# evoldoers/historian

Hardware: AMD Instinct MI355X
Metric: forward-DP cells/s (higher is better)
Workload: dtype f64; 1 GPU; batch of independent 2x2000-residue protein leaf-profile pairs, WAG, t=0.2/0.3, full (unbanded) Forward DP; scaled-probability recursion with the reference's truncation: every pairwise sum of the reference's left-nested log_sum_exp drops a term that is at most e^-10 of the other, as the reference's table does (src/logsumexp.h:45); no table, log-probabilities at the store; lpEnd within 1e-9 rel. of; pairs_per_gpu=512, pairs_total=512, parallelism=pairs farmed across 1 rank(s); RCCL broadcast of model constants only

## Files before the change

historian_amd/csrc/hx_band2.hip:

```cpp
#include <hip/hip_runtime.h>
#include <cstdlib>
#include "hx_device.h"
#include "hx_lse.h"
#include "hx_common.h"
#include "hx_policy.h"
#include "hx_kernels.h"
#include "hx_bandedge.h"

namespace hx {

namespace {

typedef double d2v __attribute__((ext_vector_type(2)));
typedef int i2v __attribute__((ext_vector_type(2)));

#define HXB2_EMIN (-(1 << 28))
#define HXB2_LOG_ENTRIES 1536
#define HXB2_HOLE_BEGIN 16
#define HXB2_HOLE_END 16384
#define HXB2_W 32
#define HXB2_INFLIGHT 30
#define HXB2_LONG_ROW 16

struct L5 { double imm, imd, idm, imi, iiw; int e; };
__device__ __forceinline__ L5 l5_zero() { return L5{0., 0., 0., 0., 0., HXB2_EMIN}; }

__device__ __forceinline__ int ror1(int v) { return __builtin_amdgcn_mov_dpp(v, 0x13C , 0xf, 0xf, false); }
__device__ __forceinline__ int rot(const int, const int v) { return ror1(ror1(v)); }
__device__ __forceinline__ double rot(const int addr, const double v) {
  return __hiloint2double(rot(addr, __double2hiint(v)), rot(addr, __double2loint(v)));
}
__device__ __forceinline__ double ror1(const double v) { return __hiloint2double(ror1(__double2hiint(v)), ror1(__double2loint(v))); }
__device__ __forceinline__ L5 rot(const int, const L5& c) {
  const L5 t{ror1(c.imm), ror1(c.imd), ror1(c.idm), ror1(c.imi), ror1(c.iiw), ror1(c.e)};
  __builtin_amdgcn_sched_barrier(0);
  const L5 r{ror1(t.imm), ror1(t.imd), ror1(t.idm), ror1(t.imi), ror1(t.iiw), ror1(t.e)};
  __builtin_amdgcn_sched_barrier(0);
  return r;
}

__device__ __forceinline__ double trunc_sum(double a, double b) {
  const double hi = fmax_plain(a, b), lo = fmin_plain(a, b);
  const int keep = lo > hi * 4.5399929762484854e-05 ? __double2hiint(lo) : 0;
  return hi + __hiloint2double(keep, __double2loint(lo));
}
template <bool TRUNC> __device__ __forceinline__ double lin_acc(double m, double p, double acc) {
  if (TRUNC) return trunc_sum(acc, m * p);
  return __builtin_fma(m, p, acc);
}

__device__ __forceinline__ double log_scaled(double m, int e) {
  const double f = __builtin_amdgcn_frexp_mant(m);
  const int k = __builtin_amdgcn_frexp_exp(m);
  const unsigned byte_off = ((unsigned)__double2hiint(f) >> 7) & 0x7FF0u;
  const d2v ce = *(const HX_LDS d2v*)(uintptr_t)byte_off;
  const double r = __builtin_fma(f, ce.x, -1.0);
  double p = __builtin_fma(r, 1.0 / 3.0, -0.5);
  p = __builtin_fma(p, r, 1.0);
  const double lf = __builtin_fma(p, r, ce.y);
  return __builtin_fma((double)(e + k), 0.693147180559945309417, lf);
}

__device__ __forceinline__ double read_lane(double v, int l) {
  return __hiloint2double(__builtin_amdgcn_readlane(__double2hiint(v), l), __builtin_amdgcn_readlane(__double2loint(v), l));
}

struct Band2Plan { int sbase, ycol, yclass, xclass, elds, stride, in_hole, total; };

__device__ __forceinline__ int block_offset(const Band2Plan& p, const int pair) {
  return pair < p.in_hole ? HXB2_HOLE_BEGIN + pair * p.stride : 16 * HXB2_LOG_ENTRIES + (pair - p.in_hole) * p.stride;
}

template <bool TRUNC, int DIR>
__global__ void __launch_bounds__(256)
k_band2_edges(const DevJob* __restrict__ jobs, const int n_jobs, const int write_edges) {
  const int lane = threadIdx.x & 63;
  const int job = (int)blockIdx.x * 4 + (int)(threadIdx.x >> 6);
  if (job >= n_jobs) return;
  const DevJob J = jobs[job];
  const int Re = J.n_rows, Ce = J.n_cols;
  const int nse = (Re + 63) >> 6;
  const int64_t plane = J.plane;
  const int blk = J.blk;
  HX_GLOBAL double* __restrict__ M = as_global(DIR ? J.bwd : J.fwd);
  const HX_GLOBAL i2v* xrecG = (const HX_GLOBAL i2v*)as_global(reinterpret_cast<const i2v*>(DIR ? J.band_rows_bwd : J.band_rows));
  if (DIR == 1) {
    const int64_t ssd = J.strip_stride;
    const int lo_last = reinterpret_cast<const int*>(reinterpret_cast<const i2v*>(J.band_rows_bwd) + (Re + 64))[nse];
    auto put_inf = [&](const int ip, const int jp) {
      const int64_t sl = cell_slot_blk(ssd, blk, ip, jp);
      M[sl] = HX_NEG_INF; M[plane + sl] = HX_NEG_INF; M[2 * plane + sl] = HX_NEG_INF; M[3 * plane + sl] = HX_NEG_INF;
      M[4 * plane + sl] = HX_NEG_INF;
    };
    if (write_edges) {
      for (int ip = 1 + lane; ip < Re; ip += 64) {
        const i2v rec = xrecG[ip];
        if ((rec.x & 0xFFFF) + ((rec.y >> 9) & 7) - ip > 0) put_inf(ip, 0);
      }
      for (int jp = 1 + lane; jp < lo_last; jp += 64) put_inf(Re - 1, jp);
    }
    {
      const i2v rec = xrecG[0];
      if (lane == 0 && (rec.x & 0xFFFF) + ((rec.y >> 9) & 7) > 0) {
        const double lpe = J.x.pack[4 * (size_t)Re] + J.y.pack[4 * (size_t)Ce];
        const int64_t sl = cell_slot_blk(ssd, blk, 0, 0);
        for (int st = 0; st < 5; ++st) M[st * plane + sl] = lpe + J.T[st][5];
      }
    }
  } else {
    const int own0 = (xrecG[0].x >> 16) & 0xFFFF;
    const i2v rec1 = xrecG[1];
    const bool row1_edge = ((rec1.x & 0xFFFF) + ((rec1.x >> 16) & 0xFFFF) - 1) < Ce - 1;
    const double T02 = J.T[0][2], T03 = J.T[0][3], T22 = J.T[2][2], T33 = J.T[3][3];
    const double pen0 = J.x.pack[3];
    double d_idm = HX_NEG_INF, d_imi = HX_NEG_INF;
    if (own0 < Ce - 1 || row1_edge) {
      const bool packed = J.strip_base != nullptr;
      const int w0 = packed ? J.fwd_windows[0] : 0, w1 = packed ? J.fwd_windows[1] : 0, w2 = packed ? J.fwd_windows[2] : 0,
                w3 = packed ? J.fwd_windows[3] : 0;
      const int64_t b0 = packed ? J.strip_base[0] : 0, b1 = packed ? J.strip_base[1] : 0;
      auto row0_slot = [&](const int j) -> int64_t {
        if (!packed) return cell_slot_blk(J.strip_stride, J.blk, 0, j);
        if (j >= w0 && j < w1) return b0 + ((int64_t)((j - w0) >> 1) << 7) + (j & 1);
        if (j >= w2 && j < w3) return b1 + ((int64_t)((j - w2) >> 1) << 7) + (j & 1);
        return -1;
      };
      const HX_GLOBAL double* ypack = as_global(J.y.pack);
      int full_from = own0 + 1;
      for (int l = 1; l < 4 && l < Re; ++l) {
        const i2v r = xrecG[l];
        if ((r.x & 0xFFFF) != 0xFFFF) full_from = max(full_from, (r.x & 0xFFFF) + ((r.x >> 16) & 0xFFFF) + 1);
      }
      full_from = (full_from + 1) & ~1;
      double carry_idm = 0., carry_imi = 0.;
      for (int j0 = 0; j0 < Ce; j0 += 64) {
        const int j = j0 + lane;
        const size_t jl = 4 * (size_t)(j < Ce ? j : Ce - 1);
        const double lrs = ypack[jl + 1], lin = ypack[jl + 2];
        double kidm, kimi;
        row0_chain_block(j0, lane, Ce, lrs, lin, T02, T03, T22, T33, pen0, carry_idm, carry_imi, kidm, kimi);
        if (Ce - 2 >= j0 && Ce - 2 < j0 + 64) { d_idm = read_lane(kidm, Ce - 2 - j0); d_imi = read_lane(kimi, Ce - 2 - j0); }
#pragma unroll
        for (int half = 0; half < 2; ++half) {
          const int line = (lane >> 2) + 16 * half, piece = lane & 3;
          const int je = j0 + 2 * line;
          const double e_idm = __shfl(kidm, 2 * line, 64), o_idm = __shfl(kidm, 2 * line + 1, 64);
          const double e_imi = __shfl(kimi, 2 * line, 64), o_imi = __shfl(kimi, 2 * line + 1, 64);
          const int64_t sl = je + 1 < Ce ? row0_slot(je) : -1;
          if (je >= full_from && sl >= 0) {
            const d2v ninf = d2v{HX_NEG_INF, HX_NEG_INF};
            HX_GLOBAL d2v* L = (HX_GLOBAL d2v*)(M + sl) + piece;
            const int64_t plane2 = plane >> 1;
            L[0] = ninf; L[plane2] = ninf; L[4 * plane2] = ninf;
            L[2 * plane2] = piece == 0 ? d2v{e_idm, o_idm} : ninf;
            L[3 * plane2] = piece == 0 ? d2v{e_imi, o_imi} : ninf;
          }
        }
        if (j > own0 && j < Ce && ((j & ~1) < full_from || (j | 1) >= Ce)) {
          const int64_t sl = row0_slot(j);
          if (sl >= 0) {
            M[sl] = HX_NEG_INF; M[plane + sl] = HX_NEG_INF; M[2 * plane + sl] = kidm; M[3 * plane + sl] = kimi; M[4 * plane + sl] = HX_NEG_INF;
          }
        }
      }
    }
    if (row1_edge) {
      double dv[5] = {HX_NEG_INF, HX_NEG_INF, HX_NEG_INF, HX_NEG_INF, HX_NEG_INF};
      if (Ce - 2 == 0) dv[0] = 0.0; else { dv[2] = d_idm; dv[3] = d_imi; }
      const unsigned c = (unsigned)J.y.ecls[Ce - 1] & 0x7Fu;
      const unsigned eo = (unsigned)(rec1.y & 0xFF) * (unsigned)(J.y.n_cls + 1);
      double acc = HX_NEG_INF;
      for (int q = 0; q < 5; ++q) {
        const double t = dv[q] + J.T[q][0];
        const double hi = vmax(acc, t), lo = vmin(acc, t);
        const bool add = hi > HX_NEG_INF && lo > HX_NEG_INF && (!TRUNC || hi - lo < 10.0);
        acc = add ? hi + log1p(exp(lo - hi)) : hi;
      }
      const double imm = acc > HX_NEG_INF ? acc + J.emis_pad[eo + c] : HX_NEG_INF;
      const int64_t sl = stored_slot(J, 1, Ce - 1);
      if (lane == 0 && sl >= 0) {
        M[sl] = imm; M[plane + sl] = HX_NEG_INF; M[2 * plane + sl] = HX_NEG_INF; M[3 * plane + sl] = HX_NEG_INF; M[4 * plane + sl] = HX_NEG_INF;
      }
    }
    if (write_edges)
      for (int i = 2 + lane; i < Re; i += 64) {
        const i2v rec = xrecG[i];
        const int last_col = (rec.x & 0xFFFF) + ((rec.x >> 16) & 0xFFFF) - i;
        if (last_col < Ce - 1) {
          const int64_t sl = stored_slot(J, i, Ce - 1);
          if (sl >= 0) {
            M[sl] = HX_NEG_INF; M[plane + sl] = HX_NEG_INF; M[2 * plane + sl] = HX_NEG_INF; M[3 * plane + sl] = HX_NEG_INF; M[4 * plane + sl] = HX_NEG_INF;
          }
        }
      }
  }
}

template <bool TRUNC, int NW, int DIR>
__global__ void __launch_bounds__(NW * 64, 2)
k_fill_band2(const DevJob* __restrict__ jobs, const double* __restrict__ exact_tab, const double* __restrict__ log_tab,
             const Band2Plan plan, const int n_jobs) {
  constexpr int THREADS = NW * 64;
  extern __shared__ __attribute__((aligned(16))) unsigned char lds[];
  const int wave = __builtin_amdgcn_readfirstlane((int)(threadIdx.x >> 6));
  const int lane = threadIdx.x & 63;
  const int half = lane & 1, r32 = lane >> 1;
  double* ptab = reinterpret_cast<double*>(lds);
  for (int k = threadIdx.x; k < 2; k += THREADS) ptab[k] = log_tab[k];
  for (int k = 2048 + threadIdx.x; k < 2 * HXB2_LOG_ENTRIES; k += THREADS) ptab[k] = log_tab[k];
  const int first_job = (int)blockIdx.x * 2 * NW;

  const int my_pair = 2 * wave + half;
  const int my_job = first_job + my_pair;
  const bool live = my_job < n_jobs;
  const DevJob* __restrict__ Jp = jobs + (my_job < n_jobs ? my_job : 0);
  unsigned char* blkp = lds + block_offset(plan, my_pair);
  HX_LDS int* sbaseL = (HX_LDS int*)(blkp + plan.sbase);
  HX_LDS unsigned char* ycolL = (HX_LDS unsigned char*)(blkp + plan.ycol);
  HX_LDS d2v* yclassL = (HX_LDS d2v*)(blkp + plan.yclass);
  HX_LDS d2v* xclassL = (HX_LDS d2v*)(blkp + plan.xclass);
  HX_LDS double* eldsL = (HX_LDS double*)(blkp + plan.elds);
  const int R = Jp->n_rows, Cc = Jp->n_cols;
  const int n_strips = (R + 63) >> 6;
  const int Ky1 = Jp->y.n_cls + 1, Kx1 = Jp->x.n_cls + 1;
  const i2v* rowsG = reinterpret_cast<const i2v*>(DIR ? Jp->band_rows_bwd : Jp->band_rows);
  if (live) {
    const int* sb = reinterpret_cast<const int*>(rowsG + (R + 64));
    for (int q = r32; q < n_strips; q += 32) sbaseL[q] = sb[q];
    for (int j = r32; j < Cc; j += 32) {
      const int jc = DIR ? Cc - 1 - j : j;
      ycolL[j] = (unsigned char)((unsigned)Jp->y.ecls[DIR ? jc + 1 : jc] | (Jp->y.pack[4 * (size_t)jc + 3] < 0.0 ? 0x80u : 0u));
    }
    for (int c = r32; c < Ky1; c += 32) {
      const bool real = c < Jp->y.n_cls;
      const int rep = real ? Jp->y.cls_rep[c] : 0;
      yclassL[c] = real ? d2v{exp(Jp->y.pack[4 * (size_t)rep + 1]), exp(Jp->y.pack[4 * (size_t)rep + 2])} : d2v{0., 0.};
    }
    for (int c = r32; c < Kx1; c += 32) {
      const bool real = c < Jp->x.n_cls;
      const int rep = real ? Jp->x.cls_rep[c] : 0;
      xclassL[c] = real ? d2v{exp(Jp->x.pack[4 * (size_t)rep + 1]), exp(Jp->x.pack[4 * (size_t)rep + 2])} : d2v{0., 0.};
    }
    for (int e = r32; e < Kx1 * Ky1; e += 32) eldsL[e] = exp(Jp->emis_pad[e]);
  }
  __syncthreads();

  {
    const int rot_addr = 0;
    const int64_t plane2 = Jp->plane >> 1;
    HX_GLOBAL double* __restrict__ M = as_global(DIR ? Jp->bwd : Jp->fwd);
    const HX_GLOBAL i2v* xrecG = (const HX_GLOBAL i2v*)as_global(rowsG);
    auto xrec_at = [&](const int i) -> i2v { return xrecG[i]; };
    i2v landing;
    asm volatile("; landing registers of the row-record fetches: %0" : "=v"(landing));
    auto xrec_fetch = [&](const int i) {
      const HX_GLOBAL i2v* a = xrecG + i;
      asm volatile("global_load_dwordx2 %0, %1, off" : : "v"(landing), "v"(a) : "memory");
    };
    auto xrec_take = [&](const bool short_row) -> i2v {
      int x, y;
      if (__builtin_amdgcn_ballot_w64(short_row) != 0)
        asm volatile("s_waitcnt vmcnt(0)\n\tv_mov_b32 %0, %2\n\tv_mov_b32 %1, %3" : "=&v"(x), "=&v"(y) : "v"(landing.x), "v"(landing.y) : "memory");
      else
        asm volatile("s_waitcnt vmcnt(%4)\n\tv_mov_b32 %0, %2\n\tv_mov_b32 %1, %3" : "=&v"(x), "=&v"(y) : "v"(landing.x), "v"(landing.y), "n"(HXB2_INFLIGHT) : "memory");
      return i2v{x, y};
    };
    const int my_steps = live ? ((DIR ? Jp->band_steps_bwd : Jp->band_steps) + 7) & ~7 : 0;
    const int s0 = __builtin_amdgcn_readlane(my_steps, 0), s1 = __builtin_amdgcn_readlane(my_steps, 1);
    const int n_steps = s0 > s1 ? s0 : s1;

    int i = r32, os, oe, as;
    unsigned span;
    HX_GLOBAL d2v* rowp;
    unsigned erow;
    unsigned ycur;
    double xc_rs, xc_in;
    int x_wait;
    i2v nrec;
    d2v nxc = d2v{0., 0.};
    int nstore = 0;
    unsigned nerow = 0;
    const unsigned ycol_lo = (unsigned)(uintptr_t)ycolL, ycol_hi = ycol_lo + (unsigned)(Cc - 1);
    const unsigned elds_a = (unsigned)(uintptr_t)eldsL, yclass_a = (unsigned)(uintptr_t)yclassL;
    auto decode = [&](const i2v r, const d2v xc, const int sb, const unsigned er) {
      os = r.x & 0xFFFF; oe = os + ((r.x >> 16) & 0xFFFF);
      as = os + ((r.y >> 9) & 7);
      span = (unsigned)((oe - ((r.y >> 12) & 7)) - as);
      if ((r.x & 0xFFFF) == 0xFFFF || !live) { os = 0x7FFFFFF0; oe = 0x7FFFFFF1; as = os; span = 1; }
      rowp = (HX_GLOBAL d2v*)(M + sb);
      erow = er;
      x_wait = (r.y & 0x100) ? (1 << 29) : 0;
      xc_rs = xc.x; xc_in = xc.y;
      ycur = ycol_lo - (unsigned)i;
    };
    auto store_base = [&](const int row) -> int { return sbaseL[row < R ? row >> 6 : 0] + 2 * (row & 63); };
    auto emis_row = [&](const i2v r) -> unsigned { return elds_a + 8u * (unsigned)(r.y & 0xFF) * (unsigned)Ky1; };
    {
      const i2v r0 = xrec_at(r32 < R ? r32 : R);
      decode(r0, xclassL[r0.y & 0xFF], store_base(r32), emis_row(r0));
      nrec = i2v{0xFFFF, 0};
      xrec_fetch(r32 + HXB2_W < R ? r32 + HXB2_W : R);
    }
    double P[5][5];
#pragma unroll
    for (int a = 0; a < 5; ++a)
#pragma unroll
      for (int d = 0; d < 5; ++d) {
        const bool used = d == 0 || (d == 1 && a != 4) || (d == 2 && a != 3) || (d == 3 && (a == 0 || a == 3)) ||
                          (d == 4 && (a == 0 || a == 3 || a == 4));
        P[a][d] = used ? exp(Jp->T[a][d]) : 0.;
      }
    double end_cell[5] = {0., 0., 0., 0., 0.};
    if (DIR == 1) {
      const double lpe = Jp->x.pack[4 * (size_t)R] + Jp->y.pack[4 * (size_t)Cc];
      for (int s = 0; s < 5; ++s) end_cell[s] = exp(lpe + Jp->T[s][5]);
    }

    L5 la = l5_zero(), lb = l5_zero(), lua = l5_zero(), lub = l5_zero();

    auto byte_at = [&](const unsigned addr) -> unsigned {
      const int a = (int)addr < (int)ycol_lo ? (int)ycol_lo : ((int)addr > (int)ycol_hi ? (int)ycol_hi : (int)addr);
      return *(const HX_LDS unsigned char*)(uintptr_t)(unsigned)a;
    };
    unsigned w_cur = byte_at(ycur), w_nxt = byte_at(ycur + 1);
    d2v rc_cur = yclassL[w_cur & 0x7Fu];
    double em_cur = *(const HX_LDS double*)(uintptr_t)(erow + 8u * (w_cur & 0x7Fu));

    auto roll_even = [&](const int k) {
      if (k > oe) {
        i += HXB2_W;
        decode(nrec, nxc, nstore, nerow);
        xrec_fetch(i + HXB2_W < R ? i + HXB2_W : R);
      }
    };
    auto roll_odd = [&](const int k) {
      if (k == oe) {
        nrec = xrec_take(oe - os < HXB2_LONG_ROW - 1);
        nxc = xclassL[nrec.y & 0xFF];
        nstore = store_base(i + HXB2_W);
        nerow = emis_row(nrec);
      }
    };
    struct YSide { unsigned w; d2v rc; double em; };
    auto y_side = [&](const int k) -> YSide {
      const YSide now{w_cur, rc_cur, em_cur};
      const unsigned c1 = w_nxt & 0x7Fu;
      rc_cur = *(const HX_LDS d2v*)(uintptr_t)(yclass_a + 16u * c1);
      em_cur = *(const HX_LDS double*)(uintptr_t)(((k + 1 > oe) ? nerow : erow) + 8u * c1);
      w_cur = w_nxt;
      w_nxt = byte_at(((oe <= k + 1) ? ycur - HXB2_W : ycur) + (unsigned)(k + 2));
      return now;
    };

    auto step = [&](const int k, const bool renorm, const L5& left, L5& out, L5& u1, L5& u2, const YSide ys) {
      const d2v rc = ys.rc;
      const int y_wait = (int)((ys.w & 0x80u) << 22);
      const double em = ys.em;
      int E = left.e > u1.e ? left.e : u1.e;
      E = E > u2.e ? E : u2.e;
      const int Eo = E + ((unsigned)(k - as) <= span ? 0 : (1 << 29));
      const int du = (u1.e - y_wait) - Eo, dl = (left.e - x_wait) - Eo, dd = u2.e - Eo;
      if (DIR == 1) {
        const double tD = u2.imm * em;
        const double t1x = u1.imd * xc_rs, t2x = u1.iiw * xc_in;
        const double t1y = left.idm * rc.x, t2y = left.imi * rc.y;
        const double D = __builtin_ldexp(tD, dd);
        const double d1x = __builtin_ldexp(t1x, du), d2x = __builtin_ldexp(t2x, du);
        const double d1y = __builtin_ldexp(t1y, dl), d2y = __builtin_ldexp(t2y, dl);
        out.imm = lin_acc<TRUNC>(P[0][3], d2y, lin_acc<TRUNC>(P[0][2], d1y, lin_acc<TRUNC>(P[0][4], d2x, lin_acc<TRUNC>(P[0][1], d1x, P[0][0] * D))));
        out.imd = lin_acc<TRUNC>(P[1][2], d1y, lin_acc<TRUNC>(P[1][1], d1x, P[1][0] * D));
        out.idm = lin_acc<TRUNC>(P[2][2], d1y, lin_acc<TRUNC>(P[2][1], d1x, P[2][0] * D));
        out.imi = lin_acc<TRUNC>(P[3][3], d2y, lin_acc<TRUNC>(P[3][4], d2x, lin_acc<TRUNC>(P[3][1], d1x, P[3][0] * D)));
        out.iiw = lin_acc<TRUNC>(P[4][2], d1y, lin_acc<TRUNC>(P[4][4], d2x, P[4][0] * D));
      } else {
        double s_imd = u1.imm * P[0][1];
        double s_iiw = u1.imm * P[0][4];
        double s_idm = left.imm * P[0][2];
        double s_imi = left.imm * P[0][3];
        double s_imm = u2.imm * P[0][0];
        s_imd = lin_acc<TRUNC>(u1.imd, P[1][1], s_imd);
        s_iiw = lin_acc<TRUNC>(u1.imi, P[3][4], s_iiw);
        s_idm = lin_acc<TRUNC>(left.imd, P[1][2], s_idm);
        s_imi = lin_acc<TRUNC>(left.imi, P[3][3], s_imi);
        s_imm = lin_acc<TRUNC>(u2.imd, P[1][0], s_imm);
        s_imd = lin_acc<TRUNC>(u1.idm, P[2][1], s_imd);
        s_iiw = lin_acc<TRUNC>(u1.iiw, P[4][4], s_iiw);
        s_idm = lin_acc<TRUNC>(left.idm, P[2][2], s_idm);
        s_imm = lin_acc<TRUNC>(u2.idm, P[2][0], s_imm);
        s_imd = lin_acc<TRUNC>(u1.imi, P[3][1], s_imd);
        s_idm = lin_acc<TRUNC>(left.iiw, P[4][2], s_idm);
        s_imm = lin_acc<TRUNC>(u2.imi, P[3][0], s_imm);
        s_imm = lin_acc<TRUNC>(u2.iiw, P[4][0], s_imm);
        out.imd = __builtin_ldexp(s_imd * xc_rs, du);
        out.iiw = __builtin_ldexp(s_iiw * xc_in, du);
        out.idm = __builtin_ldexp(s_idm * rc.x, dl);
        out.imi = __builtin_ldexp(s_imi * rc.y, dl);
        out.imm = __builtin_ldexp(s_imm * em, dd);
      }
      out.e = E;
      if (renorm) {
        if (k == 0 && r32 == 0 && live) {
          if (DIR == 0) { out.imm = 1.0; out.e = 0; }
          else {
            out.imm = end_cell[0]; out.imd = end_cell[1]; out.idm = end_cell[2]; out.imi = end_cell[3]; out.iiw = end_cell[4];
            out.e = 0;
          }
        }
        const double mx = vmax(vmax(vmax(out.imm, out.imd), vmax(out.idm, out.imi)), out.iiw);
        const int kk = __builtin_amdgcn_frexp_exp(mx);
        out.imm = __builtin_ldexp(out.imm, -kk);
        out.imd = __builtin_ldexp(out.imd, -kk);
        out.idm = __builtin_ldexp(out.idm, -kk);
        out.imi = __builtin_ldexp(out.imi, -kk);
        out.iiw = __builtin_ldexp(out.iiw, -kk);
        out.e = mx > 0. ? out.e + kk : HXB2_EMIN;
      }
      u2 = rot(rot_addr, out);
    };

    auto step_pair = [&](const int k, const bool renorm) {
      roll_even(k);
      const bool own = k >= os && k <= oe;
      HX_GLOBAL d2v* M2 = rowp + ((k >> 1) << 6);
      step(k, renorm, lb, la, lua, lub, y_side(k));
      const double l0 = log_scaled(la.imm, la.e), l1 = log_scaled(la.imd, la.e), l2 = log_scaled(la.idm, la.e),
                   l3 = log_scaled(la.imi, la.e), l4 = log_scaled(la.iiw, la.e);
      roll_odd(k + 1);
      step(k + 1, renorm, la, lb, lub, lua, y_side(k + 1));
      const double h0 = log_scaled(lb.imm, lb.e), h1 = log_scaled(lb.imd, lb.e), h2 = log_scaled(lb.idm, lb.e),
                   h3 = log_scaled(lb.imi, lb.e), h4 = log_scaled(lb.iiw, lb.e);
      if (own) {
        __builtin_nontemporal_store(d2v{l0, h0}, &M2[0]);
        __builtin_nontemporal_store(d2v{l1, h1}, &M2[plane2]);
        __builtin_nontemporal_store(d2v{l2, h2}, &M2[2 * plane2]);
        __builtin_nontemporal_store(d2v{l3, h3}, &M2[3 * plane2]);
        __builtin_nontemporal_store(d2v{l4, h4}, &M2[4 * plane2]);
      }
    };
    for (int k = 0; k < n_steps; k += 8) {
      step_pair(k, true);
      step_pair(k + 2, false);
      step_pair(k + 4, false);
      step_pair(k + 6, false);
    }
  }
  asm volatile("s_waitcnt vmcnt(0)" ::: "memory");
}

template <int DIR>
__global__ void __launch_bounds__(64)
k_band2_result(const DevJob* __restrict__ jobs, const double* __restrict__ exact_tab, const int n_jobs) {
  const int job = (int)(blockIdx.x * blockDim.x + threadIdx.x);
  if (job >= n_jobs) return;
  const DevJob& J = jobs[job];
  if (DIR == 0) *J.lp_end = forward_lp_end(J, ExactLse{exact_tab});
  else *J.lp_start = J.bwd[cell_slot_blk(J.strip_stride, J.blk, J.n_rows - 1, J.n_cols - 1)];
}

Band2Plan plan_band2(int nw, int max_rows, int max_cols, int max_cls) {
  Band2Plan p;
  int a = 0;
  p.sbase = a; a += (4 * ((max_rows + 63) / 64 + 1) + 15) & ~15;
  p.ycol = a; a += (max_cols + 15) & ~15;
  p.yclass = a; a += 16 * (max_cls + 1);
  p.xclass = a; a += 16 * (max_cls + 1);
  p.elds = a; a += (8 * (max_cls + 1) * (max_cls + 1) + 15) & ~15;
  p.stride = a;
  p.in_hole = (HXB2_HOLE_END - HXB2_HOLE_BEGIN) / a;
  if (p.in_hole > 2 * nw) p.in_hole = 2 * nw;
  p.total = 16 * HXB2_LOG_ENTRIES + (2 * nw - p.in_hole) * a;
  return p;
}

template <bool TRUNC, int NW, int DIR>
int launch_b2(const DevJob* d_jobs, int n_jobs, const Band2Plan& p, const double* tab, const double* log_tab, int write_edges, hipStream_t st,
              hipStream_t edge_st) {
  if (p.total > HX_LDS_LIMIT) return launch_fail("k_fill_band2<%d> needs %d bytes of LDS (limit %d)", NW, p.total, HX_LDS_LIMIT);
  hipLaunchKernelGGL((k_fill_band2<TRUNC, NW, DIR>), dim3((n_jobs + 2 * NW - 1) / (2 * NW)), dim3(NW * 64), p.total, st, d_jobs, tab,
                     log_tab, p, n_jobs);
  hipLaunchKernelGGL((k_band2_edges<TRUNC, DIR>), dim3((n_jobs + 3) / 4), dim3(256), 0, edge_st, d_jobs, n_jobs, write_edges);
  return 0;
}

template <int DIR>
int launch_band2_dir(const DevJob* d_jobs, int n_jobs, bool trunc, int max_rows, int max_cols, int max_cls, Tab8 tab8, Tab16 log_tab,
                     bool write_edges, hipStream_t st, hipStream_t edge_st) {
  if (max_cls + 1 > 127) return launch_fail("%d emission classes exceed the two-pairs-per-wavefront sweep's column bytes", max_cls);
  const char* v = getenv("HX_BAND2_NW");
  int nw = v ? atoi(v) : 0;
  if (nw != 1 && nw != 2 && nw != 4) nw = 4;
  const int we = write_edges ? 1 : 0;
#define HXB2_GO(NW_) do { const Band2Plan p = plan_band2(NW_, max_rows, max_cols, max_cls); \
    return trunc ? launch_b2<true, NW_, DIR>(d_jobs, n_jobs, p, tab8.p, log_tab.p, we, st, edge_st) \
                 : launch_b2<false, NW_, DIR>(d_jobs, n_jobs, p, tab8.p, log_tab.p, we, st, edge_st); } while (0)
  if (nw == 4) HXB2_GO(4);
  if (nw == 2) HXB2_GO(2);
  HXB2_GO(1);
#undef HXB2_GO
}

}

bool band2_kernel_fits(int rows, int cols, int cls) {
  return cls + 1 <= 127 && plan_band2(1, rows, cols, cls).total <= HX_LDS_LIMIT;
}

void launch_band2_result(const DevJob* d_jobs, int n_jobs, int dir, Tab8 tab8, hipStream_t st) {
  if (dir == 0) hipLaunchKernelGGL(k_band2_result<0>, dim3((n_jobs + 63) / 64), dim3(64), 0, st, d_jobs, tab8.p, n_jobs);
  else hipLaunchKernelGGL(k_band2_result<1>, dim3((n_jobs + 63) / 64), dim3(64), 0, st, d_jobs, tab8.p, n_jobs);
}

int launch_forward_band2(const DevJob* d_jobs, int n_jobs, bool trunc, int max_rows, int max_cols, int max_cls, Tab8 tab8, Tab16 log_tab,
                         bool write_edges, hipStream_t st, hipStream_t edge_st) {
  return launch_band2_dir<0>(d_jobs, n_jobs, trunc, max_rows, max_cols, max_cls, tab8, log_tab, write_edges, st, edge_st);
}
int launch_backward_band2(const DevJob* d_jobs, int n_jobs, bool trunc, int max_rows, int max_cols, int max_cls, Tab8 tab8, Tab16 log_tab,
                          bool write_edges, hipStream_t st, hipStream_t edge_st) {
  return launch_band2_dir<1>(d_jobs, n_jobs, trunc, max_rows, max_cols, max_cls, tab8, log_tab, write_edges, st, edge_st);
}

}
```

Before: 115.9 billion cells/s.

## Pre-reduce up-neighbor contributions before lane rotation and split log into issue/finish

For the forward direction, each cell now folds its outgoing contributions to the next row's match/delete/insert states into three partial sums before the DPP rotation. The rotation then moves three doubles plus an exponent instead of five doubles plus an exponent, which cuts cross-lane traffic. The log-at-store is split into an LDS table-fetch phase and a finish phase, with sched barriers, so LDS latency overlaps the next step and log work runs only for owned rows. The y-column clamp also becomes a single v_med3_i32 instruction.

Result: no change. 115.9 billion cells/s, median of 2 (-0.1%).

```diff
diff --git a/historian_amd/csrc/hx_band2.hip b/historian_amd/csrc/hx_band2.hip
--- a/historian_amd/csrc/hx_band2.hip
+++ b/historian_amd/csrc/hx_band2.hip
@@ -24,6 +24,8 @@
 
 struct L5 { double imm, imd, idm, imi, iiw; int e; };
 __device__ __forceinline__ L5 l5_zero() { return L5{0., 0., 0., 0., 0., HXB2_EMIN}; }
+struct Up { double md, iw, mm; int e; };
+__device__ __forceinline__ Up up_zero() { return Up{0., 0., 0., HXB2_EMIN}; }
 
 __device__ __forceinline__ int ror1(int v) { return __builtin_amdgcn_mov_dpp(v, 0x13C , 0xf, 0xf, false); }
 __device__ __forceinline__ int rot(const int, const int v) { return ror1(ror1(v)); }
@@ -31,10 +33,10 @@
   return __hiloint2double(rot(addr, __double2hiint(v)), rot(addr, __double2loint(v)));
 }
 __device__ __forceinline__ double ror1(const double v) { return __hiloint2double(ror1(__double2hiint(v)), ror1(__double2loint(v))); }
-__device__ __forceinline__ L5 rot(const int, const L5& c) {
-  const L5 t{ror1(c.imm), ror1(c.imd), ror1(c.idm), ror1(c.imi), ror1(c.iiw), ror1(c.e)};
+__device__ __forceinline__ Up rot(const int, const Up& c) {
+  const Up t{ror1(c.md), ror1(c.iw), ror1(c.mm), ror1(c.e)};
   __builtin_amdgcn_sched_barrier(0);
-  const L5 r{ror1(t.imm), ror1(t.imd), ror1(t.idm), ror1(t.imi), ror1(t.iiw), ror1(t.e)};
+  const Up r{ror1(t.md), ror1(t.iw), ror1(t.mm), ror1(t.e)};
   __builtin_amdgcn_sched_barrier(0);
   return r;
 }
@@ -49,11 +51,14 @@
   return __builtin_fma(m, p, acc);
 }
 
-__device__ __forceinline__ double log_scaled(double m, int e) {
+__device__ __forceinline__ d2v log_issue(double m) {
+  const double f = __builtin_amdgcn_frexp_mant(m);
+  const unsigned byte_off = ((unsigned)__double2hiint(f) >> 7) & 0x7FF0u;
+  return *(const HX_LDS d2v*)(uintptr_t)byte_off;
+}
+__device__ __forceinline__ double log_finish(double m, int e, d2v ce) {
   const double f = __builtin_amdgcn_frexp_mant(m);
   const int k = __builtin_amdgcn_frexp_exp(m);
-  const unsigned byte_off = ((unsigned)__double2hiint(f) >> 7) & 0x7FF0u;
-  const d2v ce = *(const HX_LDS d2v*)(uintptr_t)byte_off;
   const double r = __builtin_fma(f, ce.x, -1.0);
   double p = __builtin_fma(r, 1.0 / 3.0, -0.5);
   p = __builtin_fma(p, r, 1.0);
@@ -316,11 +321,13 @@
       for (int s = 0; s < 5; ++s) end_cell[s] = exp(lpe + Jp->T[s][5]);
     }
 
-    L5 la = l5_zero(), lb = l5_zero(), lua = l5_zero(), lub = l5_zero();
+    L5 la = l5_zero(), lb = l5_zero();
+    Up lua = up_zero(), lub = up_zero();
 
     auto byte_at = [&](const unsigned addr) -> unsigned {
-      const int a = (int)addr < (int)ycol_lo ? (int)ycol_lo : ((int)addr > (int)ycol_hi ? (int)ycol_hi : (int)addr);
-      return *(const HX_LDS unsigned char*)(uintptr_t)(unsigned)a;
+      unsigned a;
+      asm("v_med3_i32 %0, %1, %2, %3" : "=v"(a) : "v"(addr), "v"(ycol_lo), "v"(ycol_hi));
+      return *(const HX_LDS unsigned char*)(uintptr_t)a;
     };
     unsigned w_cur = byte_at(ycur), w_nxt = byte_at(ycur + 1);
     d2v rc_cur = yclassL[w_cur & 0x7Fu];
@@ -352,7 +359,7 @@
       return now;
     };
 
-    auto step = [&](const int k, const bool renorm, const L5& left, L5& out, L5& u1, L5& u2, const YSide ys) {
+    auto step = [&](const int k, const bool renorm, const L5& left, L5& out, const Up& u1, Up& u2, const YSide ys) {
       const d2v rc = ys.rc;
       const int y_wait = (int)((ys.w & 0x80u) << 22);
       const double em = ys.em;
@@ -361,8 +368,8 @@
       const int Eo = E + ((unsigned)(k - as) <= span ? 0 : (1 << 29));
       const int du = (u1.e - y_wait) - Eo, dl = (left.e - x_wait) - Eo, dd = u2.e - Eo;
       if (DIR == 1) {
-        const double tD = u2.imm * em;
-        const double t1x = u1.imd * xc_rs, t2x = u1.iiw * xc_in;
+        const double tD = u2.mm * em;
+        const double t1x = u1.md * xc_rs, t2x = u1.iw * xc_in;
         const double t1y = left.idm * rc.x, t2y = left.imi * rc.y;
         const double D = __builtin_ldexp(tD, dd);
         const double d1x = __builtin_ldexp(t1x, du), d2x = __builtin_ldexp(t2x, du);
@@ -373,24 +380,13 @@
         out.imi = lin_acc<TRUNC>(P[3][3], d2y, lin_acc<TRUNC>(P[3][4], d2x, lin_acc<TRUNC>(P[3][1], d1x, P[3][0] * D)));
         out.iiw = lin_acc<TRUNC>(P[4][2], d1y, lin_acc<TRUNC>(P[4][4], d2x, P[4][0] * D));
       } else {
-        double s_imd = u1.imm * P[0][1];
-        double s_iiw = u1.imm * P[0][4];
+        const double s_imd = u1.md, s_iiw = u1.iw, s_imm = u2.mm;
         double s_idm = left.imm * P[0][2];
         double s_imi = left.imm * P[0][3];
-        double s_imm = u2.imm * P[0][0];
-        s_imd = lin_acc<TRUNC>(u1.imd, P[1][1], s_imd);
-        s_iiw = lin_acc<TRUNC>(u1.imi, P[3][4], s_iiw);
         s_idm = lin_acc<TRUNC>(left.imd, P[1][2], s_idm);
         s_imi = lin_acc<TRUNC>(left.imi, P[3][3], s_imi);
-        s_imm = lin_acc<TRUNC>(u2.imd, P[1][0], s_imm);
-        s_imd = lin_acc<TRUNC>(u1.idm, P[2][1], s_imd);
-        s_iiw = lin_acc<TRUNC>(u1.iiw, P[4][4], s_iiw);
         s_idm = lin_acc<TRUNC>(left.idm, P[2][2], s_idm);
-        s_imm = lin_acc<TRUNC>(u2.idm, P[2][0], s_imm);
-        s_imd = lin_acc<TRUNC>(u1.imi, P[3][1], s_imd);
         s_idm = lin_acc<TRUNC>(left.iiw, P[4][2], s_idm);
-        s_imm = lin_acc<TRUNC>(u2.imi, P[3][0], s_imm);
-        s_imm = lin_acc<TRUNC>(u2.iiw, P[4][0], s_imm);
         out.imd = __builtin_ldexp(s_imd * xc_rs, du);
         out.iiw = __builtin_ldexp(s_iiw * xc_in, du);
         out.idm = __builtin_ldexp(s_idm * rc.x, dl);
@@ -415,7 +411,24 @@
         out.iiw = __builtin_ldexp(out.iiw, -kk);
         out.e = mx > 0. ? out.e + kk : HXB2_EMIN;
       }
-      u2 = rot(rot_addr, out);
+      Up h;
+      if (DIR == 1) { h.md = out.imd; h.iw = out.iiw; h.mm = out.imm; }
+      else {
+        h.md = out.imm * P[0][1];
+        h.iw = out.imm * P[0][4];
+        h.mm = out.imm * P[0][0];
+        h.md = lin_acc<TRUNC>(out.imd, P[1][1], h.md);
+        h.iw = lin_acc<TRUNC>(out.imi, P[3][4], h.iw);
+        h.mm = lin_acc<TRUNC>(out.imd, P[1][0], h.mm);
+        h.md = lin_acc<TRUNC>(out.idm, P[2][1], h.md);
+        h.iw = lin_acc<TRUNC>(out.iiw, P[4][4], h.iw);
+        h.mm = lin_acc<TRUNC>(out.idm, P[2][0], h.mm);
+        h.md = lin_acc<TRUNC>(out.imi, P[3][1], h.md);
+        h.mm = lin_acc<TRUNC>(out.imi, P[3][0], h.mm);
+        h.mm = lin_acc<TRUNC>(out.iiw, P[4][0], h.mm);
+      }
+      h.e = out.e;
+      u2 = rot(rot_addr, h);
     };
 
     auto step_pair = [&](const int k, const bool renorm) {
@@ -423,13 +436,19 @@
       const bool own = k >= os && k <= oe;
       HX_GLOBAL d2v* M2 = rowp + ((k >> 1) << 6);
       step(k, renorm, lb, la, lua, lub, y_side(k));
-      const double l0 = log_scaled(la.imm, la.e), l1 = log_scaled(la.imd, la.e), l2 = log_scaled(la.idm, la.e),
-                   l3 = log_scaled(la.imi, la.e), l4 = log_scaled(la.iiw, la.e);
+      const d2v ea0 = log_issue(la.imm), ea1 = log_issue(la.imd), ea2 = log_issue(la.idm), ea3 = log_issue(la.imi),
+                ea4 = log_issue(la.iiw);
       roll_odd(k + 1);
       step(k + 1, renorm, la, lb, lub, lua, y_side(k + 1));
-      const double h0 = log_scaled(lb.imm, lb.e), h1 = log_scaled(lb.imd, lb.e), h2 = log_scaled(lb.idm, lb.e),
-                   h3 = log_scaled(lb.imi, lb.e), h4 = log_scaled(lb.iiw, lb.e);
       if (own) {
+        const d2v eb0 = log_issue(lb.imm), eb1 = log_issue(lb.imd), eb2 = log_issue(lb.idm), eb3 = log_issue(lb.imi),
+                  eb4 = log_issue(lb.iiw);
+        __builtin_amdgcn_sched_barrier(0);
+        const double l0 = log_finish(la.imm, la.e, ea0), l1 = log_finish(la.imd, la.e, ea1), l2 = log_finish(la.idm, la.e, ea2),
+                     l3 = log_finish(la.imi, la.e, ea3), l4 = log_finish(la.iiw, la.e, ea4);
+        __builtin_amdgcn_sched_barrier(0);
+        const double h0 = log_finish(lb.imm, lb.e, eb0), h1 = log_finish(lb.imd, lb.e, eb1), h2 = log_finish(lb.idm, lb.e, eb2),
+                     h3 = log_finish(lb.imi, lb.e, eb3), h4 = log_finish(lb.iiw, lb.e, eb4);
         __builtin_nontemporal_store(d2v{l0, h0}, &M2[0]);
         __builtin_nontemporal_store(d2v{l1, h1}, &M2[plane2]);
         __builtin_nontemporal_store(d2v{l2, h2}, &M2[2 * plane2]);
```
